# Equim-chan/Mortal

Hardware: AMD Instinct MI355X
Metric: env steps/sec (65536 parallel tables per GPU) (higher is better)
Workload: dtype u8/i32 state, f32 obs

## Files before the change

include/mortal_amd.h:

```cpp
#ifndef MORTAL_AMD_H
#define MORTAL_AMD_H

#include <stddef.h>
#include <stdint.h>

#ifdef __cplusplus
extern "C" {
#endif

typedef struct MjPool MjPool;

enum { MJ_DEAL_RAND08 = 0, MJ_DEAL_RAND09 = 1 };

const char* mj_last_error(void);
int mj_abi_version(void);

int mj_tables_upload(const void* payload, size_t size);

MjPool* mj_pool_create(int n_tables, int version, int deal_algo, int max_rows);
void mj_pool_destroy(MjPool* pool);

int mj_pool_reset(MjPool* pool, const uint64_t* nonces, const uint64_t* keys, const uint32_t* game_ids,
                  const uint8_t* agent_of_seat, int n_games_total);

// ... 15 lines not shown

int mj_replay_load(MjPool* pool, const uint64_t* script_host, const uint32_t* off_host, const uint8_t* tracked_host,
                   int n_logs, int always_include_kan_select, const uint64_t* nonces_host ,
                   const uint64_t* keys_host );
#define MJ_LOAD_DEAL_FROM_SEED 1
#define MJ_LOAD_AUGMENT 2
int mj_replay_load_pool(MjPool* dst, MjPool* src, int table0, const uint8_t* tracked_host ,
                        int always_include_kan_select, int flags , int64_t counts_out[3], void* stream);
int mj_replay_step(MjPool* pool, void* stream);
int mj_replay_meta(MjPool* pool, int32_t* meta_dev, void* stream);

int mj_table_apply_event(MjPool* pool, int table, const uint64_t* words_host, int n_words, void* stream);
int mj_table_mark_row(MjPool* pool, int table, int seat, int at_kan_select, void* stream);
int mj_table_query(MjPool* pool, int table, int seat, int what, const int32_t* args8_host, int32_t* out8_host, void* stream);

int mj_rows_count(MjPool* pool, int32_t n_rows_out[2], void* stream);
const uint32_t* mj_rows_dev(MjPool* pool, int agent);

int mj_encode(MjPool* pool, int agent, float* obs_dev, uint8_t* masks_dev, void* stream);
int mj_encode_oracle(MjPool* pool, int agent, float* out_dev, void* stream);
int mj_oracle_obs_rows(int version);
int mj_encode_timing(MjPool* pool, int enable, double* total_ms_out, int64_t* launches_out);
int mj_sp_timing(MjPool* pool, double* total_ms_out, int64_t* launches_out);
int mj_sp_phase_ticks(MjPool* pool, uint64_t* out8, void* stream);
int mj_pool_set_sp_schedule(MjPool* pool, int mode, int max_rows, int wide_grid, int min_level1, int min_level2);
int mj_sp_schedule_stats(MjPool* pool, uint64_t* out4, void* stream);

int mj_random_policy(MjPool* pool, int agent, const uint8_t* masks_dev, uint64_t seed, uint64_t cycle,
                     int32_t* actions_dev, void* stream);

int mj_greedy_policy(MjPool* pool, int agent, const uint8_t* masks_dev, const float* obs_dev, uint64_t seed, uint64_t cycle,
                     int32_t* actions_dev, void* stream);

int mj_counters(MjPool* pool, uint64_t out[8], void* stream);
int mj_results(MjPool* pool, int32_t* scores_out, uint8_t* done_out, void* stream);
#define MJ_STAT_FIELDS 44
enum MjStatField {
    MJ_ST_GAME = 0, MJ_ST_ROUND, MJ_ST_OYA, MJ_ST_POINT, MJ_ST_RANK_1, MJ_ST_RANK_2, MJ_ST_RANK_3, MJ_ST_RANK_4, MJ_ST_TOBI,
    MJ_ST_FUURO, MJ_ST_FUURO_NUM, MJ_ST_FUURO_POINT, MJ_ST_FUURO_AGARI, MJ_ST_FUURO_AGARI_JUN, MJ_ST_FUURO_AGARI_POINT,
    MJ_ST_FUURO_HOUJUU, MJ_ST_AGARI, MJ_ST_AGARI_AS_OYA, MJ_ST_AGARI_JUN, MJ_ST_AGARI_POINT_OYA, MJ_ST_AGARI_POINT_KO,
    MJ_ST_HOUJUU, MJ_ST_HOUJUU_JUN, MJ_ST_HOUJUU_TO_OYA, MJ_ST_HOUJUU_POINT_TO_OYA, MJ_ST_HOUJUU_POINT_TO_KO,
    MJ_ST_RIICHI, MJ_ST_RIICHI_AS_OYA, MJ_ST_RIICHI_JUN, MJ_ST_RIICHI_AGARI, MJ_ST_RIICHI_AGARI_POINT, MJ_ST_RIICHI_AGARI_JUN,
    MJ_ST_RIICHI_HOUJUU, MJ_ST_RIICHI_RYUKYOKU, MJ_ST_RIICHI_POINT, MJ_ST_CHASING_RIICHI, MJ_ST_RIICHI_GOT_CHASED,
    MJ_ST_DAMA_AGARI, MJ_ST_DAMA_AGARI_JUN, MJ_ST_DAMA_AGARI_POINT, MJ_ST_RYUKYOKU, MJ_ST_RYUKYOKU_POINT, MJ_ST_YAKUMAN,
    MJ_ST_NAGASHI_MANGAN
};
int mj_stat_logs(const uint64_t* words_host, const uint32_t* off_host , int n_logs,
// ... 66 lines not shown
```

mortal_amd/csrc/mj_capi.hip:

```cpp
#include <hip/hip_runtime.h>

#include <algorithm>
#include <cmath>
#include <cstdio>
#include <cstring>
#include <functional>
#include <memory>
#include <optional>
#include <string>
#include <vector>

#include "../../include/mortal_amd.h"
#include "mj_host.h"
#include "mj_step.hip"
#include "mj_replay.hip"
#include "mj_encode.hip"
#include "mj_sp.hip"
#include "mj_stat.hip"
#include "mj_gameplay.hip"
#include "mj_harvest.hip"

static_assert(sizeof(MjAlgoQuery) == 72, "MjAlgoQuery layout");
__global__ __launch_bounds__(64) void mj_k_algo_query(const MjAlgoQuery* q, int n, MjAlgoResult* out) {
    const int i = blockIdx.x * 64 + threadIdx.x;
// ... 692 lines not shown
    return kp;
}

static int sp_setup(MjPool* P, int agent, float* obs, hipStream_t s) {
    SpResources R;
    const PoolKnobs& K = P->knobs;
    if (R.err.alloc(SP_ERR_WORDS)) return -1;
    HIP_OK(hipMemset(R.err.get(), 0, SP_ERR_WORDS * sizeof(unsigned long long)));
    if (R.order.alloc(P->max_rows) || R.cls.alloc(P->max_rows)) return -1;
    R.grid = std::min(256 * SP_WGS, P->max_rows);
    if (K.sp_grid) R.grid = std::max(1, std::min(R.grid, *K.sp_grid));
    const bool env = !P->sp_sched_set;
    const int wide_mode = env && K.sp_wide ? *K.sp_wide : P->sp_wide_mode;
    const int wide_max_rows = env && K.sp_wide_max_rows ? *K.sp_wide_max_rows : P->sp_wide_max_rows;
    R.spare = wide_mode == 0 ? 0 : std::min(SP_PROMO_CAP, std::max(8, P->n_tables / 4) & ~1);
    if (wide_mode < 0 && P->n_tables > wide_max_rows) R.spare = 0;
    R.wide_areas = R.spare ? std::min(256, std::max(2, P->n_tables / 16)) : 0;
    const int areas = R.grid + R.spare + R.wide_areas;
    if (R.work.alloc(areas)) return -1;
    for (int g = 0; g < areas; g++) {
        SpWork& W = R.work.get()[g];
        HIP_OK(hipMemsetAsync(W.tag, 0, sizeof(W.tag), s));
        HIP_OK(hipMemsetAsync(&W.epoch, 0, sizeof(W.epoch) + sizeof(W.pad_), s));
    }
    if (R.queue.alloc(SP_Q_WORDS)) return -1;
    if (R.spare) {
        if (R.stream2.create_non_blocking() || R.ev_fork.create_no_timing() || R.ev_join.create_no_timing() || R.gaveup_host.alloc(1)) return -1;
        *R.gaveup_host.get() = 0ull;
        HIP_OK(hipMemsetAsync(R.queue.get(), 0, SP_Q_WORDS * sizeof(int), s));
        HIP_OK(hipStreamSynchronize(s));
        SpParams w = sp_params(P, R, agent, obs, 0);
        w.sweep = 1;
        hipLaunchKernelGGL(mj_k_sp_wide, dim3(1), dim3(SP_WIDE_THREADS), 0, s, w);
        hipLaunchKernelGGL(mj_k_sp_promo, dim3(1), dim3(SP_THREADS), 0, R.stream2.get(), w);
        HIP_OK(hipStreamSynchronize(R.stream2.get()));
        HIP_OK(hipStreamSynchronize(s));
        HIP_OK(hipGetLastError());
    }
    P->sp = std::move(R);
    P->sp_wide_mode = wide_mode;
    P->sp_wide_max_rows = wide_max_rows;
    if (env && K.sp_wide_grid) P->sp_wide_grid = std::max(1, *K.sp_wide_grid);
    if (env && K.sp_promo_min1) P->sp_promo_min[1] = std::max(1, *K.sp_promo_min1);
    if (env && K.sp_promo_min2) P->sp_promo_min[2] = std::max(1, *K.sp_promo_min2);
    return 0;
}
// ... 209 lines not shown
                    sp_[8], sp_[0], sp_[1], sp_[2], sp_[3], sp_[4], sp_[9], sp_[5], sp_[10], sp_[7]);
            for (int k = 11; k < 32; k++) fprintf(stderr, " %llu", sp_[k]);
            fprintf(stderr, "\n");
        }
    }
#endif
    if (!P) return fail("null pool");
    HIP_OK(hipStreamSynchronize((hipStream_t)stream));
    unsigned long long tmp[8];
    HIP_OK(hipMemcpy(tmp, P->counters.get(), sizeof tmp, hipMemcpyDeviceToHost));
    for (int i = 0; i < 8; i++) out[i] = tmp[i];
    out[5] = P->cycles;
    int f = 0;
    HIP_OK(hipMemcpy(&f, P->enc_flag.get(), sizeof f, hipMemcpyDeviceToHost));
    out[6] = (unsigned long long)f;
    if (P->sp.err) {
        unsigned long long e2[SP_ERR_WORDS];
        HIP_OK(hipMemcpy(e2, P->sp.err.get(), sizeof e2, hipMemcpyDeviceToHost));
        out[6] += e2[SP_ERR_OVERFLOW];
        out[7] = e2[SP_ERR_ROWS];
        const unsigned long long* pass = e2 + SP_ERR_PASS;
        if (P->knobs.sp_prof)
            fprintf(stderr, "[sp prof] rows %llu setup %llu expand %llu evalL0 %llu evalL>0 %llu encode %llu states %llu (wall_clock64 ticks, 100 MHz) | "
                    "expand passes: probes %llu lists+V %llu td-probes %llu layout %llu inserts %llu; items %llu expanded %llu edges %llu l0-entries %llu; level-0 probe %llu scoring %llu; workgroup lifetimes: sum %llu max %llu queue pops %llu hash resets %llu; eval wavefront time %llu; shader clock %.0f MHz (s_memtime cycles %llu over the lifetimes)\n",
                    e2[SP_ERR_ROWS], e2[SP_ERR_T_SETUP], e2[SP_ERR_T_EXPAND], e2[SP_ERR_T_EVAL0], e2[SP_ERR_T_EVAL], e2[SP_ERR_T_WRITE], e2[SP_ERR_STATES],
                    pass[0], pass[1], pass[2], pass[3], pass[4], pass[5], pass[6], e2[SP_ERR_EDGES], e2[SP_ERR_L0_ITEMS],
                    e2[SP_ERR_T_L0_PROBE], e2[SP_ERR_T_L0_SCORE], e2[SP_ERR_WG_LIFE], e2[SP_ERR_WG_LIFE_MAX], e2[SP_ERR_T_POP], e2[SP_ERR_T_RESET],
                    e2[SP_ERR_T_EVAL_WAVE], e2[SP_ERR_WG_LIFE] ? 100.0 * (double)e2[SP_ERR_WG_CLOCK] / (double)e2[SP_ERR_WG_LIFE] : 0.0,
                    e2[SP_ERR_WG_CLOCK]);
    }
    return 0;
}

#ifdef MJ_EMU
void mj_emu_sp_placed(uint64_t out[2]) { out[0] = g_sp_emu_placed[0]; out[1] = g_sp_emu_placed[1]; }
void mj_emu_sp_lost_claims(uint64_t out[4]) {
    for (int k = 0; k < 2; k++) out[k] = g_sp_emu_lost[2 + k], out[2 + k] = g_sp_emu_lost[k] - g_sp_emu_lost[2 + k];
}
#ifdef MJ_EMU_REGISTRY
void mj_emu_alloc_stats(uint64_t out[6]) {
    const emu::Registry& r = emu::R();
    out[0] = r.buffers.size(), out[1] = r.events.size(), out[2] = r.streams.size(), out[3] = r.bad_frees, out[4] = r.allocs, out[5] = r.syncs;
}
void mj_emu_fail_nth(int alloc, int sync) { emu::R().fail_alloc_in = alloc, emu::R().fail_sync_in = sync; }
#endif
#endif

int mj_sp_phase_ticks(MjPool* P, uint64_t out[8], void* stream) {
    if (!P) return fail("null pool");
    for (int i = 0; i < 8; i++) out[i] = 0;
    if (!P->sp.err) return 0;
    HIP_OK(hipStreamSynchronize((hipStream_t)stream));
    unsigned long long e2[8];
    HIP_OK(hipMemcpy(e2, P->sp.err.get(), sizeof e2, hipMemcpyDeviceToHost));
    for (int i = 0; i < 8; i++) out[i] = e2[i];
    return 0;
}

int mj_pool_set_sp_schedule(MjPool* P, int mode, int max_rows, int wide_grid, int min_level1, int min_level2) {
    if (!P) return fail("null pool");
    if (P->sp.work && mode != 0 && mode >= -1 && P->sp.spare == 0) return fail("mj_pool_set_sp_schedule: the work areas are allocated (call it before the first obs-v4 mj_encode)");
    if (mode >= -1) P->sp_wide_mode = mode > 0 ? 1 : mode;
    if (max_rows > 0) P->sp_wide_max_rows = max_rows;
    if (wide_grid > 0) P->sp_wide_grid = std::min(wide_grid, 256);
    if (min_level1 > 0) P->sp_promo_min[1] = min_level1;
    if (min_level2 > 0) P->sp_promo_min[2] = min_level2;
    P->sp_sched_set = true;
    return 0;
}

int mj_sp_schedule_stats(MjPool* P, uint64_t out[4], void* stream) {
    if (!P) return fail("null pool");
    for (int i = 0; i < 4; i++) out[i] = 0;
    if (!P->sp.err) return 0;
    HIP_OK(hipStreamSynchronize((hipStream_t)stream));
    unsigned long long e2[SP_ERR_WORDS];
    HIP_OK(hipMemcpy(e2, P->sp.err.get(), sizeof e2, hipMemcpyDeviceToHost));
    out[0] = P->sp_hybrid_launches;
// ... 462 lines not shown
```

mortal_amd/csrc/mj_sp.hip:

```cpp
#include <hip/hip_runtime.h>

#include <type_traits>
#ifdef MJ_EMU
#include <algorithm>
#endif

#include "mj_rules.h"
#include "mj_sptab.h"


#ifndef SP_THREADS
#define SP_THREADS 256
#endif
#define SP_CAP 16384
#define SP_T 17
#define SP_MAX_CAND 14
#ifndef SP_NS
#define SP_NS 16
#endif
#ifndef SP_SORT_MIN
#define SP_SORT_MIN 8
#endif
#ifndef SP_ITEM_CAP
#define SP_ITEM_CAP 64
#endif
#ifndef SP_WPS
#define SP_WPS 4
#endif
#define SP_WGS (4 * SP_WPS * 64 / SP_THREADS)

#ifndef SP_SET_BUCKETS
#define SP_SET_BUCKETS 1024
#endif
#define SP_SET_SLOTS (2 * SP_SET_BUCKETS)
#define SP_NODES (SP_CAP + SP_SET_SLOTS)
static_assert((SP_SET_BUCKETS & (SP_SET_BUCKETS - 1)) == 0 && SP_SET_BUCKETS >= 1 && SP_NODES <= (1 << 15), "slots are 15-bit fields");
#ifndef SP_TAIL_BATCH
#define SP_TAIL_BATCH 4
#endif
#define SP_Q_TAIL 32
#define SP_Q_PROMO_DONE 96
#define SP_PROMO_LEVELS 2
#define SP_Q_PROMO_ALLOC(p) (128 + 64 * (p))
#define SP_Q_PROMO_HEAD(p) (160 + 64 * (p))
#define SP_Q_PROMO_ENT 256
#ifndef SP_PROMO_CAP
#define SP_PROMO_CAP 512
#endif
#define SP_Q_WORDS (SP_Q_PROMO_ENT + SP_PROMO_CAP)
#ifndef SP_WIDE_THREADS
#define SP_WIDE_THREADS 1024
#endif
#define SP_POOL (SP_CAP * 32)
#define SP_ITEMS (SP_CAP * 4)
#define SP_L0_MAX 17
#define SP_EL_SLOT(v) ((v) & 0x7FFFu)
#define SP_EL_IDX(v) ((v) >> 15)
struct alignas(128) SpNode {
    float val[SP_T][3];
// ... 1 lines not shown
};
static_assert(sizeof(SpNode) == 256 && offsetof(SpNode, val) == 0, "SpNode layout");
struct alignas(16) SpHdr {
    u32 child_off;
    unsigned short n_ch;
    u8 sumreq, n_ent;
    u64 l0cnt2;
};
static_assert(sizeof(SpHdr) == 16 && offsetof(SpHdr, n_ch) == 4 && offsetof(SpHdr, sumreq) == 6 && offsetof(SpHdr, l0cnt2) == 8,
              "the evaluation reads the header as one or two u64");
struct SpKeys {
    u64 k0, k1, k2, k3;
    u64 dk;
};
#define SP_ENT_SLOT(e) ((e) & 0x7FFFu)
#define SP_ENT_KEY(e) (((e) >> 15) & 511u)
#define SP_ENT_LAST (1u << 24)
#define SP_ENT_COUNT(e) (((e) >> 25) & 7u)
#define SP_ENT_INVALID (1u << 28)
struct alignas(16) SpF4 { float x, y, z, w; };
#define SP_HANDOFF_WORDS 1024
struct alignas(128) SpWork {
    u64 tag[SP_CAP];
    SpNode node[SP_NODES];
    SpKeys keys[SP_CAP];
    SpHdr hdr[SP_CAP];
    u32 list[SP_CAP];
    u32 elist[SP_CAP];
    u32 pool[SP_POOL];
    u32 items[SP_ITEMS];
    SpF4 l0sc[SP_ITEMS];
    u32 epoch;
    u32 pad_[31];
    alignas(16) u32 handoff[SP_HANDOFF_WORDS];
#ifdef MJ_EMU
    u32 idx_of[SP_NODES];
#endif
};
static_assert(offsetof(SpWork, node) % 128 == 0 && sizeof(SpWork) % 128 == 0, "nodes on line boundaries");

#define SP_NT_ROWS 124
#define SP_NT_STRIDE (SP_T + 3)
__constant__ const float* c_sp_nt;
static inline void sp_not_tsumo_build(float* out ) {
    for (int n_left = 0; n_left < SP_NT_ROWS; n_left++)
        for (int q = 0; q < SP_NT_ROWS; q++) {
            float* r = out + ((size_t)n_left * SP_NT_ROWS + q) * SP_NT_STRIDE;
// ... 35 lines not shown
    SP_ERR_T_EVAL0 = 4,
    SP_ERR_T_EVAL = 5,
    SP_ERR_T_WRITE = 6,
    SP_ERR_STATES = 7,
    SP_ERR_PASS = 8,
    SP_ERR_EDGES = 15,
    SP_ERR_L0_ITEMS = 16,
    SP_ERR_T_L0_PROBE = 17,
    SP_ERR_T_L0_SCORE = 18,
    SP_ERR_WG_LIFE = 19,
    SP_ERR_WG_LIFE_MAX = 20,
    SP_ERR_T_POP = 21,
    SP_ERR_T_RESET = 22,
    SP_ERR_T_EVAL_WAVE = 23,
    SP_ERR_WG_CLOCK = 24,
    SP_ERR_STATS = 25,
    SP_ERR_WIDE_GAVEUP = 25,
    SP_ERR_PROMOTED = 26,
    SP_ERR_SWEPT = 27,
    SP_ERR_DUMP_T0 = 28,
    SP_ERR_DUMP_NARROW = 29,
    SP_ERR_DUMP_WIDE = 30,
    SP_ERR_DUMP_TAIL = 31,
    SP_ERR_WORDS = 32
};

__device__ static const float SP_URADORA[5][13] = {
    {0.639485f, 0.327801f, 0.0327134f, 0.f, 0.f, 0.f, 0.f, 0.f, 0.f, 0.f, 0.f, 0.f, 0.f},
    {0.406736f, 0.42281f, 0.147966f, 0.021674f, 0.0008142f, 0.f, 0.f, 0.f, 0.f, 0.f, 0.f, 0.f, 0.f},
    {0.257516f, 0.406819f, 0.246851f, 0.0757724f, 0.0122266f, 0.0008004f, 1.43e-5f, 0.f, 0.f, 0.f, 0.f, 0.f, 0.f},
    {0.162199f, 0.346513f, 0.301539f, 0.142396f, 0.0401276f, 0.0066491f, 0.0005575f, 1.85e-5f, 0.f, 0.f, 0.f, 0.f, 0.f},
    {0.101768f, 0.275319f, 0.313742f, 0.20189f, 0.081774f, 0.0215394f, 0.0035918f, 0.0003607f, 1.52e-5f, 3e-7f, 0.f, 0.f, 0.f}};
__device__ static const u8 SP_DISCARD_PRIO[38] = {
    6, 5, 4, 3, 2, 3, 4, 5, 6, 6, 5, 4, 3, 2, 3, 4, 5, 6, 6, 5, 4, 3, 2, 3, 4, 5, 6, 7, 7, 7, 7, 7, 7, 7, 1, 1, 1, 0};
constexpr __host__ __device__ int sp_discard_prio(int t) {
    return t < 27 ? 2 + (t % 9 > 4 ? t % 9 - 4 : 4 - t % 9) : t < 34 ? 7 : t < 37 ? 1 : 0;
}
constexpr bool sp_discard_prio_matches_table() {
    constexpr int tab[38] = {6, 5, 4, 3, 2, 3, 4, 5, 6, 6, 5, 4, 3, 2, 3, 4, 5, 6, 6, 5, 4, 3, 2, 3, 4, 5, 6, 7, 7, 7, 7, 7, 7, 7, 1, 1, 1, 0};
    for (int t = 0; t < 38; t++)
        if (sp_discard_prio(t) != tab[t]) return false;
    return true;
}
static_assert(sp_discard_prio_matches_table(), "sp_discard_prio != SP_DISCARD_PRIO");
MJD int sp_discard_key(int t) { return sp_discard_prio(t) * 64 + (63 - t); }
MJD int cmp_discard_priority(int l, int r) {
    int pl = SP_DISCARD_PRIO[l], pr = SP_DISCARD_PRIO[r];
// ... 76 lines not shown
    return *reinterpret_cast<const Tv*>(reinterpret_cast<const char*>(base) + byte_off);
#else
    return *reinterpret_cast<const SP_HBM Tv*>(reinterpret_cast<const SP_HBM char*>(base) + (unsigned long long)byte_off);
#endif
}
template <class Bp> __device__ __forceinline__ SpF4 sp_ld4(Bp base, u32 byte_off) {
#ifdef MJ_EMU
    return *reinterpret_cast<const SpF4*>(reinterpret_cast<const char*>(base) + byte_off);
#else
    const SP_HBM SpF4* p = reinterpret_cast<const SP_HBM SpF4*>(reinterpret_cast<const SP_HBM char*>(base) + (unsigned long long)byte_off);
    SpF4 r;
    r.x = p->x; r.y = p->y; r.z = p->z; r.w = p->w;
    return r;
#endif
}
struct SpF3 { float x, y, z; };
template <class Bp> __device__ __forceinline__ SpF3 sp_ld3(Bp base, u32 byte_off) {
#ifdef MJ_EMU
    return *reinterpret_cast<const SpF3*>(reinterpret_cast<const char*>(base) + byte_off);
#else
    const SP_HBM SpF3* p = reinterpret_cast<const SP_HBM SpF3*>(reinterpret_cast<const SP_HBM char*>(base) + (unsigned long long)byte_off);
    SpF3 r;
    r.x = p->x; r.y = p->y; r.z = p->z;
    return r;
#endif
}
template <class Bp> __device__ __forceinline__ void sp_st3(Bp base, u32 byte_off, float x, float y, float z) {
#ifdef MJ_EMU
    *reinterpret_cast<SpF3*>(reinterpret_cast<char*>(base) + byte_off) = SpF3{x, y, z};
#else
    SP_HBM SpF3* p = reinterpret_cast<SP_HBM SpF3*>(reinterpret_cast<SP_HBM char*>(base) + (unsigned long long)byte_off);
    p->x = x; p->y = y; p->z = z;
#endif
}
MJD int sp_f2i(float v) {
#if defined(MJ_EMU)
    return v != v ? 0 : v >= 2147483648.f ? 2147483647 : v <= -2147483648.f ? (-2147483647 - 1) : (int)v;
#else
    return (int)v;
#endif
}

MJD u64 sp_dk_add(u64 dk, int draw_tile, int discard_tile) {
    u32 d0 = (u32)dk & 63, d1 = (u32)(dk >> 6) & 63, d2 = (u32)(dk >> 12) & 63;
    u32 x0 = (u32)(dk >> 18) & 63, x1 = (u32)(dk >> 24) & 63, x2 = (u32)(dk >> 30) & 63, x3 = (u32)(dk >> 36) & 63;
    if (draw_tile >= 0) {
// ... 570 lines not shown
                Hand g = S.h;
                g.inc(t);
                kept = sp_keep_brute_dev(g, ld3, L - 1);
            } else {
                const u32 id1 = spt_id(TG, st, key1);
                const SpRec o1 = spt_opt(TG, ld3, (u32)C->r3[s][st], id1);
                u64 keepN = (u64)spt_keep_tiles(spt_rec(TG, st, key1, 1), o1) << (9 * st);
#pragma unroll
                for (int q = 0; q < 3; q++) {
                    const int u = q + (q >= st);
                    const u32 others = spt_merge(TG, (u32)C->r2[s][5 - sh_pair_idx(st, u)], id1);
                    const SpRec o = spt_opt(TG, ld3, others, (u32)C->id[s][u]);
                    keepN |= (u64)spt_keep_tiles(C->keep[s][u], o) << (9 * u);
                }
                const int yao = (int)((YAOKYUU_MASK >> t) & 1);
                SpCountSets cs;
                cs.c1 = C->cs[s][0];
                cs.c2 = C->cs[s][1];
                cs.nz = C->cs[s][2];
                kept = sp_keep_set(ld3, L - 1, spt_fin(o1), keepN, (int)C->cnt[s][0] + (hc == 1), (int)C->cnt[s][1] + (hc == 0),
                                   (int)C->cnt[s][2] + (yao && hc == 1), (int)C->cnt[s][3] + (yao && hc == 0), sp_count_sets_add(cs, t, hc));
            }
            kept &= ~(1ull << t);
            C->kept[tid] = kept;
        }
        if (prof) tp2 = wall_clock64();
        int n_entries;
        {
            const int wc = has_item ? S.w.get(my_t) : 0;
            const int nvar = has_item && sp_aka_in_wall(S, my_t) ? (wc >= 2 ? 2 : 1) : 1;
            const int nkeep = __popcll(kept), my_ent = nvar * nkeep;
            const u32 pv = sp_wave_scan_incl(has_item ? ((u32)my_ent | ((u32)wc << 16) | ((u32)(nkeep ? nvar : 0) << 24)) : 0u);
            const int sfn = __shfl((pre_ex - base) | (nt_lane << 16), has_item ? my_s : sb);
            const int s_first = sfn & 0xFFFF, s_n = sfn >> 16;
            const int s_last = s_first + s_n - 1;
            const u32 before = __shfl(pv, max(s_first - 1, 0)), upto = __shfl(pv, max(s_last, 0)), all = __shfl(pv, SP_NT - 1);
            const u32 base = s_first > 0 ? before : 0u;
            n_entries = (int)(all & 0xFFFFu);
            if (has_item) {
                C->coff[tid] = (unsigned short)(((pv - base) & 0xFFFFu) - (u32)my_ent);
                const int e_first = (int)((pv & 0xFFFFu) - (u32)my_ent);
                C->eoff[tid] = (unsigned short)e_first;
                {
                    int r = 0;
                    for (u64 rest = kept; rest; rest &= rest - 1, r++) {
                        const u32 d = (u32)(__ffsll((long long)rest) - 1);
// ... 156 lines not shown
        mj_team_sync<SP_NT>();
        if (prof) {
            tp4 = wall_clock64();
            acc_list += tp1 - tp0;
            acc_keep += tp2 - tp1;
            acc_layout += tp3 - tp2;
            acc_ins += tp4 - tp3;
            n_items_total += n_items;
            n_edges_total += n_entries;
        }
        sb = se;
    }
    if (prof && tid == 0) {
        atomicAdd(&X->pt[0], (unsigned long long)t_probe);
        atomicAdd(&X->pt[1], (unsigned long long)acc_list);
        atomicAdd(&X->pt[2], (unsigned long long)acc_keep);
        atomicAdd(&X->pt[3], (unsigned long long)acc_layout);
        atomicAdd(&X->pt[4], (unsigned long long)acc_ins);
        atomicAdd(&X->pt[5], (unsigned long long)n_items_total);
        atomicAdd(&X->pt[6], (unsigned long long)n);
    }
}

#define SP_EVAL_LDS_FLOATS(NT) (((NT) / 64) * 1408)

#define SP_EV_ENT 4
#define SP_EVW_WAVE_FLOATS 1408
MJD int sp_evw_team_floats(int T) { return SP_EV_ENT * (T + 4) * 4; }
__device__ static const u8 SP_EVW_STRIDE[SP_T + 1][4] = {
    {16, 16, 16, 16}, {20, 20, 20, 20}, {25, 25, 24, 24}, {29, 28, 29, 28}, {32, 32, 32, 32}, {37, 36, 38, 38}, {42, 41, 44, 41}, {44, 44, 44, 44},
    {48, 50, 50, 50}, {57, 56, 55, 54}, {58, 57, 56, 56}, {67, 66, 69, 60}, {68, 67, 66, 69}, {77, 68, 69, 70}, {78, 77, 76, 75}, {79, 78, 77, 76},
    {80, 86, 86, 85}, {97, 84, 86, 86}};
#define SP_EV0_STRIDE 28
#define SP_EV0_SC 20
#define SP_EV0_LAST 24

template <int TN>
__device__ SP_ATTR_EVAL0 void sp_eval_wave0(SpWork* W, SpCtx* X, float* WL, int first, int end, int stride, int lane_in_team, int off_,
                                           int team_in_wave, bool team_on) {
    SP_ASSUME_LDS(X);
    SP_ASSUME_LDS(WL);
    SP_HBM SpWork* const Wg = (SP_HBM SpWork*)sp_uniform(W);
    SP_HBM SpNode* const nodeB = sp_uniform(&Wg->node[0]);
    SP_HBM u32* const elistB = sp_uniform(&Wg->elist[0]);
    const int T = __builtin_amdgcn_readfirstlane(X->T), off = __builtin_amdgcn_readfirstlane(off_);
    const int ln = min(lane_in_team + off, SP_T - 1);
// ... 127 lines not shown
    static_assert(LK >= 1, "level 0 has no children: sp_eval_wave0");
    SP_ASSUME_LDS(X);
    SP_ASSUME_LDS(WL);
    SP_HBM SpWork* const Wg = (SP_HBM SpWork*)sp_uniform(W);
    const int T = __builtin_amdgcn_readfirstlane(X->T), off = __builtin_amdgcn_readfirstlane(off_);
    const int ln = min(lane_in_team + off, SP_T - 1);
    const int rows = T + 4;
    const int team_rows = __builtin_amdgcn_readfirstlane((int)SP_EVW_STRIDE[min(max(T, 0), SP_T)][min(max(off, 0), 3)]);
    float* const eb = WL + (team_on ? team_in_wave : 0) * (team_rows * 4);
    if (team_on)
        for (int r = lane_in_team; r < SP_EV_ENT * rows; r += T - off) *reinterpret_cast<SpF4*>(eb + 4 * r) = SpF4{0.f, 0.f, 0.f, 0.f};
    const float tp0 = X->tsumo_prob[0][ln], tp1 = X->tsumo_prob[1][ln], tp2 = X->tsumo_prob[2][ln], tp3 = X->tsumo_prob[3][ln];
    const SP_HBM float* const nt_rows = (const SP_HBM float*)c_sp_nt + (size_t)__builtin_amdgcn_readfirstlane(min(X->n_left, SP_NT_ROWS - 1)) * (SP_NT_ROWS * SP_NT_STRIDE);
    const int last = max(end - 1, 0);
    const u32 val_ln = (u32)offsetof(SpNode, val) + (u32)ln * 12u;
    SP_HBM SpNode* const nodeB = sp_uniform(&Wg->node[0]);
    SP_HBM u32* const elistB = sp_uniform(&Wg->elist[0]);
    SP_HBM u32* const poolB = sp_uniform(&Wg->pool[0]);
    SP_HBM SpHdr* const hdrB = sp_uniform(&Wg->hdr[0]);
    auto ld_slot = [&](int i) -> u32 { return sp_ld<u32>(elistB, 4u * (u32)min(i, last)); };
    auto ld_hdr = [&](u32 el) -> u64 { return sp_ld<unsigned long long>(hdrB, 16u * SP_EL_IDX(el)); };
    auto ld_m = [&](u64 hdr) -> float { return sp_ld<float>(nt_rows, 4u * ((u32)min((int)((hdr >> 48) & 0xFF), SP_NT_ROWS - 1) * SP_NT_STRIDE + (u32)ln)); };
    auto ld_ent = [&](u32 at) -> u32 { return sp_ld<u32>(poolB, 4u * min(at, (u32)(SP_POOL - 1))); };
    auto ld_val = [&](u32 ent) -> SpF3 { return sp_ld3(nodeB, SP_ENT_SLOT(ent) * (u32)sizeof(SpNode) + val_ln); };
    mj_team_sync<64>();

    int i = first;
    bool has = team_on && i < end;
    u32 s0 = ld_slot(i), s1 = ld_slot(i + stride), s2 = ld_slot(i + 2 * stride), s3 = ld_slot(i + 3 * stride);
    u64 h0 = ld_hdr(s0), h1 = ld_hdr(s1), h2 = ld_hdr(s2);
    float m_raw = ld_m(h0), m_nxt = ld_m(h1);
    u32 ent[SP_EV_ENT], entn[SP_EV_ENT], nent[SP_EV_ENT];
#pragma unroll
    for (int q = 0; q < SP_EV_ENT; q++) {
        ent[q] = ld_ent((u32)h0 + q);
        entn[q] = ld_ent((u32)h0 + SP_EV_ENT + q);
        nent[q] = ld_ent((u32)h1 + q);
    }
    SpF3 v[SP_EV_ENT];
#pragma unroll
    for (int q = 0; q < SP_EV_ENT; q++) v[q] = ld_val(ent[q]);

    int c0 = 0;
    float my_m = m_raw != 0.f ? m_raw : 1.f, my_r = sp_rcp_refined(my_m);
    float acc_t = 0.f, acc_w = 0.f, acc_e = 0.f;
    float nx_t = -3.40282347e+38f, nx_w = -3.40282347e+38f, nx_e = -3.40282347e+38f;
    int max_pack = -1;
    float* const row0 = eb + ln * 4;
    const int nl = T - ln;

    while (__ballot(has) != 0ull) {
        const int n_ch = (int)((h0 >> 32) & 0xFFFF);
        int k = 0, koff = 0;
#pragma unroll
        for (int q = 0; q < SP_EV_ENT; q++) {
            const u32 e = ent[q];
            const bool valid = has && c0 + q < n_ch;
            const bool bad = (e & SP_ENT_INVALID) != 0;
            if (valid && bad) X->overflow = 1;
            const int pack = (sp_f2i(v[q].z) << 9) | (int)SP_ENT_KEY(e);
#ifdef MJ_EMU
            if (valid && !bad && lane_in_team > 0 && ((unsigned)sp_f2i(v[q].z) >> 22)) X->overflow = 1;
#endif
            const bool better = valid && !bad && pack > max_pack;
            nx_t = better ? v[q].x : nx_t;
            nx_w = better ? v[q].y : nx_w;
            nx_e = better ? v[q].z : nx_e;
            max_pack = better ? pack : max_pack;
            if (valid && (e & SP_ENT_LAST)) {
                const u32 cnt = SP_ENT_COUNT(e);
                const float tpc = cnt <= 1 ? tp0 : cnt == 2 ? tp1 : cnt == 3 ? tp2 : tp3;
                float* row = row0 + koff;
                row[0] = nx_t;
                row[1] = nx_w;
                row[2] = nx_e;
                row[7] = tpc * m_raw;
                k++;
                koff += rows * 4;
                nx_t = nx_w = nx_e = -3.40282347e+38f;
                max_pack = -1;
            }
        }
        c0 += SP_EV_ENT;
        const bool done = has && c0 >= n_ch;
        u32 up[SP_EV_ENT], upn[SP_EV_ENT], nent2[SP_EV_ENT];
        SpF3 vn[SP_EV_ENT];
        const u32 up_off = done ? (u32)h1 + SP_EV_ENT : (u32)h0 + (u32)c0 + SP_EV_ENT;
#pragma unroll
        for (int q = 0; q < SP_EV_ENT; q++) up[q] = done ? nent[q] : entn[q];
#pragma unroll
        for (int q = 0; q < SP_EV_ENT; q++) vn[q] = ld_val(up[q]);
#pragma unroll
        for (int q = 0; q < SP_EV_ENT; q++) upn[q] = ld_ent(up_off + q);
        float m_n2 = 0.f;
        u64 h3 = 0ull;
        u32 s4 = 0u;
// ... 319 lines not shown
            for (int i = 0; i < 5; i++) X.dora_ind[i] = i < X.n_dora ? F1(dora_ind, i) : T_UNK;
            int nf = 0;
            if (!(X.is_menzen && F1(ankan_n, p) == 0)) {
                int fn = F1(fuuro_n, p);
                for (int k = 0; k < fn; k++)
                    for (int j = 0; j < 4; j++) {
                        int t = F3(fuuro, p, k, j);
                        if (t != MJ_NONE) nf += dora_factor(L, deaka(t)) + (is_aka(t) ? 1 : 0);
                    }
                int na = F1(ankan_n, p);
                for (int k = 0; k < na; k++) {
                    int t = F2(ankan, p, k);
                    nf += 4 * dora_factor(L, t) + ((t == T_5M || t == T_5P || t == T_5S) ? 1 : 0);
                }
            }
            X.num_doras_in_fuuro = nf & 0xFF;
            X.prefer_riichi = F1(scores, p) >= 1000;
            X.calc_double_riichi = can_discard0 && (F1(pflags, p) & PF_CAN_W_RIICHI) != 0;
            X.calc_haitei = calc_haitei;
            X.T = T;
            X.n_left = n_left;
            X.n_list = 0;
            X.n_pool = 0;
            X.overflow = 0;
            X.prof = prof;
            for (int k = 0; k < 8; k++) X.pt[k] = 0;
            for (int l = 0; l < 5; l++) X.lvl_begin[l] = X.lvl_end[l] = 0;
        }
        if (with_probs) {
            for (int q = tid; q < 4 * SP_T; q += NT) {
                int i = q / SP_T, j = q % SP_T;
                X.tsumo_prob[i][j] = j < T ? (float)(i + 1) / (float)(n_left - j) : 0.f;
            }
        }

        const SpTabG TG = sp_tab_g(c_sp_tab);
        if (tid >= SPEC && tid < SPEC + 34) {
            const int d = tid - SPEC;
            if (can_discard) {
                if (root.h.get(d)) {
                    Hand hc = root.h;
                    hc.dec(d);
                    X.spec_req[0][d] = sp_req_of_hand(TG, c_mj_tables, hc, ld3, cur_shanten);
                    if (cur_shanten > 3) X.spec_req[1][d] = sp_req_of_hand(TG, c_mj_tables, hc, ld3, cur_shanten + 1);
                }
            } else if (d == 0) {
// ... 196 lines not shown
#define SP_ACQUIRE_AGENT() ((void)0)
#define SP_SPIN_PAUSE() ((void)0)
#endif

#ifdef SP_ROWDUMP
#define SP_DUMP(P) ((P).rowdump != nullptr)
#else
#define SP_DUMP(P) false
#endif
template <int NT>
struct SpLds {
    union Teams {
        TableOne st;
        SpChunk wchunk[NT / SP_NT];
        float ev[SP_EVAL_LDS_FLOATS(NT)];
        SpWaveArea wave[NT / 64];
    };
};

template <int NT, bool WIDE, bool PROMO>
__device__ __forceinline__ void sp_kernel_body(SpParams P) {
    __shared__ SpCtx X;
    __shared__ int s_row, s_k;
    __shared__ unsigned long long s_stat[SP_ERR_STATS];
    if (threadIdx.x < SP_ERR_STATS) s_stat[threadIdx.x] = 0ull;
    __shared__ typename SpLds<NT>::Teams s_tm;
    constexpr bool LDS_SET = !WIDE && !PROMO;
    __shared__ __attribute__((aligned(16))) u64 s_set[SP_SET_SLOTS];
    for (int i = threadIdx.x; i < SP_SET_SLOTS; i += NT) s_set[i] = 0ull;
    unsigned n_graph_rows = 0;
    SpWork* W = WIDE ? P.work + P.n_narrow + P.promo_cap + blockIdx.x : P.work + blockIdx.x;
    SpWork* const W_own = W;
    const int tid_wg = threadIdx.x, tid = tid_wg;

    unsigned tag_epoch = W->epoch;
    unsigned own_epoch = tag_epoch;
    bool main_done = false, drained = false;

    const long long t_wg_in = SP_DUMP(P) ? wall_clock64() : 0;
    const long long t_wg0 = P.prof ? wall_clock64() : 0;
#ifndef MJ_EMU
    const long long c_wg0 = P.prof ? clock64() : 0;
#endif
    long long t_pop = 0, t_reset = 0;
    const int n_heavy = P.n_rows - P.queue[1 + 7];
    bool wave_mode = false;
    for (;;) {
        const int tid = SP_OPQ(2, tid_wg);
// ... 157 lines not shown
                                    SpHandoff* H = reinterpret_cast<SpHandoff*>(W->handoff);
                                    H->R = R;
                                    H->row = row;
                                    H->next_lv = lv;
                                    W->epoch = tag_epoch;
                                    if (SP_DUMP(P)) P.rowdump[(size_t)row * 12 + 8] = (uint32_t)t_0, P.rowdump[(size_t)row * 12 + 9] = (uint32_t)wall_clock64();
                                }
                            }
                            SP_DRAIN_STORES();
                            __syncthreads();
                            if (tid == 0) {
                                SP_RELEASE_AGENT();
                                __hip_atomic_store(P.queue + SP_Q_PROMO_ENT + pq * (SP_PROMO_CAP / SP_PROMO_LEVELS) + k, (int)(W - P.work) + 1, __ATOMIC_RELAXED,
                                                   __HIP_MEMORY_SCOPE_AGENT);
                            }
                            W = P.work + gridDim.x + pq * (P.promo_cap / SP_PROMO_LEVELS) + k;
                            tag_epoch = W->epoch;
                            parked = true;
                            break;
                        }
                    }
                }
                const int ns = min(SP_NS, max(1, (e - b + NT / SP_NT - 1) / (NT / SP_NT)));
                for (int c0 = b + ns * (tid / SP_NT); c0 < e; c0 += ns * (NT / SP_NT))
                    sp_expand_chunk<LDS_SET>(W, &X, &s_tm.wchunk[tid / SP_NT], c0, min(ns, e - c0), lv);
                __syncthreads();
                if (tid == 0) {
                    X.lvl_begin[lv - 1] = e;
                    X.lvl_end[lv - 1] = min(X.n_list, SP_CAP);
                }
                __syncthreads();
            }
            t_2 = wall_clock64();
#ifdef MJ_EMU
            if (tid == 0 && !parked) sp_emu_check_unique(W, &X);
#endif
            if (!parked)
            for (int lv = 0; lv <= cur_shanten; lv++) {
                const int b = X.lvl_begin[lv], e = X.lvl_end[lv];
                if (lv == 0) {
                    if (tid == 0) X.n_items = 0;
                    __syncthreads();
                    const int ns = min(SP_NS, max(1, (e - b + NT / SP_NT - 1) / (NT / SP_NT)));
                    for (int c0 = b + ns * (tid / SP_NT); c0 < e; c0 += ns * (NT / SP_NT))
                        sp_l0_probe_chunk(W, &X, &s_tm.wchunk[tid / SP_NT], c0, min(ns, e - c0));
                    __syncthreads();
                    const long long t_2a = wall_clock64();
                    const int n_items = min(X.n_items, SP_ITEMS);
                    if ((tid & ~63) < n_items) sp_l0_score_all(W, &X, n_items, tid, NT);
                    __syncthreads();
                    if (P.prof && tid == 0) {
                        X.pt[7] += (unsigned long long)(t_2a - t_2);
                        s_stat[SP_ERR_T_L0_SCORE] += (unsigned long long)(wall_clock64() - t_2a);
                    }
                }
                sp_sort_level<NT>(W, reinterpret_cast<int*>(s_tm.ev), b, e);
                {
                    const int off = min(cur_shanten - lv, T - 1), TW = T - off;
                    const int wl = tid & 63, tw = wl / TW, ln = wl - tw * TW;
                    float* wl_lds = s_tm.ev + (tid >> 6) * SP_EVW_WAVE_FLOATS;
                    const long long t_ev0 = P.prof ? wall_clock64() : 0;
// ... 14 lines not shown
                            if (lv == 1) sp_eval_wave<8, 1>(W, &X, wl_lds, b + team2, e, n_teams2, ln, off, tw, on);
                            else sp_eval_wave<8, 2>(W, &X, wl_lds, b + team2, e, n_teams2, ln, off, tw, on);
                        } else if (T <= 16) {
                            if (lv == 1) sp_eval_wave<16, 1>(W, &X, wl_lds, b + team2, e, n_teams2, ln, off, tw, on);
                            else sp_eval_wave<16, 2>(W, &X, wl_lds, b + team2, e, n_teams2, ln, off, tw, on);
                        } else {
                            if (lv == 1) sp_eval_wave<17, 1>(W, &X, wl_lds, b + team2, e, n_teams2, ln, off, tw, on);
                            else sp_eval_wave<17, 2>(W, &X, wl_lds, b + team2, e, n_teams2, ln, off, tw, on);
                        }
                    }
                    if (P.prof && (tid & 63) == 0) atomicAdd(&s_stat[SP_ERR_T_EVAL_WAVE], (unsigned long long)(wall_clock64() - t_ev0));
                }
                __syncthreads();
                if (lv == 0) t_3 = wall_clock64();
            }
            t_4 = wall_clock64();
        }

        if (!parked) sp_row_write<false, NT>(W->node, X, R, tid, out, s_tm.ev);
        __syncthreads();
        if (tid == 0) {
            long long t_5 = wall_clock64();
            if (!parked) s_stat[SP_ERR_ROWS] += 1ull;
            s_stat[SP_ERR_T_SETUP] += (unsigned long long)(t_1 - t_0);
            if (with_probs) {
                s_stat[SP_ERR_T_EXPAND] += (unsigned long long)(t_2 - t_1);
                if (!parked) {
                    s_stat[SP_ERR_T_EVAL0] += (unsigned long long)(t_3 - t_2);
                    s_stat[SP_ERR_T_EVAL] += (unsigned long long)(t_4 - t_3);
                    s_stat[SP_ERR_T_WRITE] += (unsigned long long)(t_5 - t_4);
                    s_stat[SP_ERR_STATES] += (unsigned long long)X.n_list;
                    s_stat[SP_ERR_EDGES] += (unsigned long long)X.n_pool;
                    s_stat[SP_ERR_L0_ITEMS] += (unsigned long long)X.n_items;
                }
                if (P.prof)
                    for (int k = 0; k < 7; k++) s_stat[SP_ERR_PASS + k] += X.pt[k];
                if (P.prof) s_stat[SP_ERR_T_L0_PROBE] += X.pt[7];
            }
            if (SP_DUMP(P) && !parked) {
                uint32_t* d = P.rowdump + (size_t)row * 12;
                int nreq = 0;
                for (int c = 0; c < n_cand; c++) nreq += X.cand_nreq[c];
                d[0] = (uint32_t)(WIDE ? 0x40000000 | (promoted ? 0x20000000 : 0) : s_row); d[1] = (uint32_t)(cur_shanten | T << 8 | n_cand << 16 | (int)can_discard << 24); d[2] = (uint32_t)nreq;
                d[3] = with_probs ? (uint32_t)X.n_list : 0u; d[4] = with_probs ? (uint32_t)X.n_pool : 0u; d[5] = with_probs ? (uint32_t)X.n_items : 0u;
                d[6] = (uint32_t)(t_5 - t_0);
                if (!promoted) d[8] = (uint32_t)t_0, d[9] = 0u;
// ... 16 lines not shown
            W->epoch = tag_epoch;
            if (PROMO && P.promo_cap > 0) {
                SP_DRAIN_STORES();
                __hip_atomic_fetch_add(P.queue + SP_Q_PROMO_DONE, 1, __ATOMIC_RELAXED, __HIP_MEMORY_SCOPE_AGENT);
            }
        }
    }
    if (P.prof && tid == 0) {
        const unsigned long long life = (unsigned long long)(wall_clock64() - t_wg0);
        s_stat[SP_ERR_WG_LIFE] += life;
#ifndef MJ_EMU
        s_stat[SP_ERR_WG_CLOCK] += (unsigned long long)(clock64() - c_wg0);
#endif
        atomicMax(&P.err[SP_ERR_WG_LIFE_MAX], life);
        s_stat[SP_ERR_T_POP] += (unsigned long long)t_pop;
        s_stat[SP_ERR_T_RESET] += (unsigned long long)t_reset;
    }
    __syncthreads();
    if (SP_DUMP(P) && tid == 0) {
        atomicMin(&P.err[SP_ERR_DUMP_T0], (unsigned long long)t_wg_in);
        atomicMax(&P.err[WIDE ? SP_ERR_DUMP_WIDE : SP_ERR_DUMP_NARROW], (unsigned long long)wall_clock64());
    }
    if (tid < SP_ERR_STATS && tid != SP_ERR_WG_LIFE_MAX && s_stat[tid]) atomicAdd(&P.err[tid], s_stat[tid]);
    if constexpr (!WIDE) {
    if (wave_mode) {
        const int wv = tid >> 6, lane = tid & 63;
        unsigned long long w_rows = 0, w_ticks = 0, w_over = 0;
        for (;;) {
            int q = 0;
            if (lane == 0) q = n_heavy + atomicAdd(P.queue + SP_Q_TAIL, SP_TAIL_BATCH);
            q = __shfl(q, 0);
            if (q >= P.n_rows) break;
            const int qe = min(q + SP_TAIL_BATCH, P.n_rows);
            for (; q < qe; q++) {
                const unsigned long long r = sp_light_row(P.rows, P.snap, P.obs, W, &s_tm.wave[wv], (int)P.order[q]);
                w_rows++;
                w_ticks += r & 0x7FFFFFFFFFFFFFFFull;
                w_over += r >> 63;
            }
        }
        if (lane == 0 && w_rows) {
            atomicAdd(&P.err[SP_ERR_ROWS], w_rows);
            atomicAdd(&P.err[SP_ERR_T_SETUP], w_ticks);
            if (w_over) atomicAdd(&P.err[SP_ERR_OVERFLOW], w_over);
        }
        if (SP_DUMP(P) && lane == 0) atomicMax(&P.err[SP_ERR_DUMP_TAIL], (unsigned long long)wall_clock64());
// ... 8 lines not shown
```

mortal_amd/pool.py:

```python
import ctypes as C

import numpy as np
import torch

from . import tables
from ._lib import MortalAmdError, check, lib

OBS_ROWS = {1: 938, 2: 942, 3: 934, 4: 1012}
ACTION_SPACE = 46
DEAL_RAND08, DEAL_RAND09 = 0, 1


def default_deal_algo():
    import os

    v = os.environ.get("MORTAL_AMD_DEAL_ALGO", "rand09").strip().lower()
    if v in ("0", "rand08", "rand0.8", "0.8"):
        return DEAL_RAND08
    if v in ("1", "rand09", "rand0.9", "0.9", "0.9.1"):
        return DEAL_RAND09
    raise ValueError(f"MORTAL_AMD_DEAL_ALGO={v!r}: expected rand08 or rand09")

_tables_ready = False

# ... 360 lines not shown
        scores = np.zeros((self.n_games_total, 4), dtype=np.int32)
        done = np.zeros(self.n_games_total, dtype=np.uint8)
        check(self._L.mj_results(self.h, scores.ctypes.data, done.ctypes.data, self._stream()))
        return scores, done

    def first_error(self):
        t = C.c_int(-1)
        code = check(self._L.mj_pool_first_error(self.h, C.byref(t), self._stream()))
        return code, t.value

    def encode_timing(self, enable=True):
        ms = C.c_double(0)
        n = C.c_int64(0)
        check(self._L.mj_encode_timing(self.h, int(enable), C.byref(ms), C.byref(n)))
        return ms.value, n.value

    def sp_timing(self):
        ms = C.c_double(0)
        n = C.c_int64(0)
        check(self._L.mj_sp_timing(self.h, C.byref(ms), C.byref(n)))
        return ms.value, n.value

    def sp_phase_ticks(self):
        out = (C.c_uint64 * 8)()
        check(self._L.mj_sp_phase_ticks(self.h, out, self._stream()))
        return dict(zip(("overflow", "rows", "setup", "expand", "level0", "eval", "write", "states"), (int(x) for x in out)))

    def set_sp_schedule(self, mode=-2, max_rows=0, wide_grid=0, min_level1=0, min_level2=0):
        check(self._L.mj_pool_set_sp_schedule(self.h, mode, max_rows, wide_grid, min_level1, min_level2))

    def sp_schedule_stats(self):
        out = (C.c_uint64 * 4)()
        check(self._L.mj_sp_schedule_stats(self.h, out, self._stream()))
        return dict(zip(("hybrid_launches", "rows_promoted", "rows_swept", "wide_gave_up"), (int(x) for x in out)))

    def debug_table(self, table):
        size = self._L.mj_debug_table_size()
        buf = (C.c_uint8 * size)()
        check(self._L.mj_debug_table(self.h, table, buf, size, self._stream()))
        raw = bytes(buf)
        out = {}
        for ent in self._L.mj_debug_layout().decode().strip(";").split(";"):
            name, size, count, off = ent.split(":")
            size, count, off = int(size), int(count), int(off)
            dt = {1: np.uint8, 2: np.uint16, 4: np.int32, 8: np.uint64}[size]
            out[name] = np.frombuffer(raw, dtype=dt, count=count, offset=off).copy()
        return out


# ... 7 lines not shown
```

Measured before the change: 4.449 million.

## Short-circuit dead leaf expansion at max tsumo depth via shared zero node

When level 1 is the last tsumo level (T equals current shanten), children can never reach a win. Instead of the full sp_expand_chunk, a lightweight dead-chunk expander points every child entry at a shared zero-initialised node slot, and level-0 evaluation is skipped for such rows. For LK==1 the eval also loads two floats instead of three and skips writing the unused first field. The change adds a counter for these rows and a ninth profiling output, and depends on the zero slot staying zero and on the claim that those leaves contribute nothing.

```diff
diff --git a/include/mortal_amd.h b/include/mortal_amd.h
--- a/include/mortal_amd.h
+++ b/include/mortal_amd.h
@@ -61,7 +61,7 @@
 int mj_oracle_obs_rows(int version);
 int mj_encode_timing(MjPool* pool, int enable, double* total_ms_out, int64_t* launches_out);
 int mj_sp_timing(MjPool* pool, double* total_ms_out, int64_t* launches_out);
-int mj_sp_phase_ticks(MjPool* pool, uint64_t* out8, void* stream);
+int mj_sp_phase_ticks(MjPool* pool, uint64_t* out9, void* stream);
 int mj_pool_set_sp_schedule(MjPool* pool, int mode, int max_rows, int wide_grid, int min_level1, int min_level2);
 int mj_sp_schedule_stats(MjPool* pool, uint64_t* out4, void* stream);
 
diff --git a/mortal_amd/csrc/mj_capi.hip b/mortal_amd/csrc/mj_capi.hip
--- a/mortal_amd/csrc/mj_capi.hip
+++ b/mortal_amd/csrc/mj_capi.hip
@@ -738,6 +738,7 @@
         SpWork& W = R.work.get()[g];
         HIP_OK(hipMemsetAsync(W.tag, 0, sizeof(W.tag), s));
         HIP_OK(hipMemsetAsync(&W.epoch, 0, sizeof(W.epoch) + sizeof(W.pad_), s));
+        HIP_OK(hipMemsetAsync(&W.node[SP_ZERO_SLOT], 0, sizeof(SpNode), s));
     }
     if (R.queue.alloc(SP_Q_WORDS)) return -1;
     if (R.spare) {
@@ -993,12 +994,12 @@
         const unsigned long long* pass = e2 + SP_ERR_PASS;
         if (P->knobs.sp_prof)
             fprintf(stderr, "[sp prof] rows %llu setup %llu expand %llu evalL0 %llu evalL>0 %llu encode %llu states %llu (wall_clock64 ticks, 100 MHz) | "
-                    "expand passes: probes %llu lists+V %llu td-probes %llu layout %llu inserts %llu; items %llu expanded %llu edges %llu l0-entries %llu; level-0 probe %llu scoring %llu; workgroup lifetimes: sum %llu max %llu queue pops %llu hash resets %llu; eval wavefront time %llu; shader clock %.0f MHz (s_memtime cycles %llu over the lifetimes)\n",
+                    "expand passes: probes %llu lists+V %llu td-probes %llu layout %llu inserts %llu; items %llu expanded %llu edges %llu l0-entries %llu; level-0 probe %llu scoring %llu; workgroup lifetimes: sum %llu max %llu queue pops %llu hash resets %llu; eval wavefront time %llu; shader clock %.0f MHz (s_memtime cycles %llu over the lifetimes); dead-leaf rows %llu\n",
                     e2[SP_ERR_ROWS], e2[SP_ERR_T_SETUP], e2[SP_ERR_T_EXPAND], e2[SP_ERR_T_EVAL0], e2[SP_ERR_T_EVAL], e2[SP_ERR_T_WRITE], e2[SP_ERR_STATES],
                     pass[0], pass[1], pass[2], pass[3], pass[4], pass[5], pass[6], e2[SP_ERR_EDGES], e2[SP_ERR_L0_ITEMS],
                     e2[SP_ERR_T_L0_PROBE], e2[SP_ERR_T_L0_SCORE], e2[SP_ERR_WG_LIFE], e2[SP_ERR_WG_LIFE_MAX], e2[SP_ERR_T_POP], e2[SP_ERR_T_RESET],
                     e2[SP_ERR_T_EVAL_WAVE], e2[SP_ERR_WG_LIFE] ? 100.0 * (double)e2[SP_ERR_WG_CLOCK] / (double)e2[SP_ERR_WG_LIFE] : 0.0,
-                    e2[SP_ERR_WG_CLOCK]);
+                    e2[SP_ERR_WG_CLOCK], e2[SP_ERR_DEAD_LEAF]);
     }
     return 0;
 }
@@ -1017,14 +1018,15 @@
 #endif
 #endif
 
-int mj_sp_phase_ticks(MjPool* P, uint64_t out[8], void* stream) {
-    if (!P) return fail("null pool");
-    for (int i = 0; i < 8; i++) out[i] = 0;
+int mj_sp_phase_ticks(MjPool* P, uint64_t out[9], void* stream) {
+    if (!P) return fail("null pool");
+    for (int i = 0; i < 9; i++) out[i] = 0;
     if (!P->sp.err) return 0;
     HIP_OK(hipStreamSynchronize((hipStream_t)stream));
-    unsigned long long e2[8];
+    unsigned long long e2[SP_ERR_WORDS];
     HIP_OK(hipMemcpy(e2, P->sp.err.get(), sizeof e2, hipMemcpyDeviceToHost));
     for (int i = 0; i < 8; i++) out[i] = e2[i];
+    out[8] = e2[SP_ERR_DEAD_LEAF];
     return 0;
 }
 
diff --git a/mortal_amd/csrc/mj_sp.hip b/mortal_amd/csrc/mj_sp.hip
--- a/mortal_amd/csrc/mj_sp.hip
+++ b/mortal_amd/csrc/mj_sp.hip
@@ -34,7 +34,8 @@
 #endif
 #define SP_SET_SLOTS (2 * SP_SET_BUCKETS)
 #define SP_NODES (SP_CAP + SP_SET_SLOTS)
-static_assert((SP_SET_BUCKETS & (SP_SET_BUCKETS - 1)) == 0 && SP_SET_BUCKETS >= 1 && SP_NODES <= (1 << 15), "slots are 15-bit fields");
+#define SP_ZERO_SLOT SP_NODES
+static_assert((SP_SET_BUCKETS & (SP_SET_BUCKETS - 1)) == 0 && SP_SET_BUCKETS >= 1 && SP_ZERO_SLOT < (1 << 15), "slots are 15-bit fields");
 #ifndef SP_TAIL_BATCH
 #define SP_TAIL_BATCH 4
 #endif
@@ -82,7 +83,7 @@
 #define SP_HANDOFF_WORDS 1024
 struct alignas(128) SpWork {
     u64 tag[SP_CAP];
-    SpNode node[SP_NODES];
+    SpNode node[SP_NODES + 1];
     SpKeys keys[SP_CAP];
     SpHdr hdr[SP_CAP];
     u32 list[SP_CAP];
@@ -164,7 +165,8 @@
     SP_ERR_DUMP_NARROW = 29,
     SP_ERR_DUMP_WIDE = 30,
     SP_ERR_DUMP_TAIL = 31,
-    SP_ERR_WORDS = 32
+    SP_ERR_DEAD_LEAF = 32,
+    SP_ERR_WORDS = 33
 };
 
 __device__ static const float SP_URADORA[5][13] = {
@@ -287,6 +289,17 @@
     const SP_HBM SpF3* p = reinterpret_cast<const SP_HBM SpF3*>(reinterpret_cast<const SP_HBM char*>(base) + (unsigned long long)byte_off);
     SpF3 r;
     r.x = p->x; r.y = p->y; r.z = p->z;
+    return r;
+#endif
+}
+struct SpF2 { float x, y; };
+template <class Bp> __device__ __forceinline__ SpF2 sp_ld2(Bp base, u32 byte_off) {
+#ifdef MJ_EMU
+    return *reinterpret_cast<const SpF2*>(reinterpret_cast<const char*>(base) + byte_off);
+#else
+    const SP_HBM SpF2* p = reinterpret_cast<const SP_HBM SpF2*>(reinterpret_cast<const SP_HBM char*>(base) + (unsigned long long)byte_off);
+    SpF2 r;
+    r.x = p->x; r.y = p->y;
     return r;
 #endif
 }
@@ -903,6 +916,9 @@
                                    (int)C->cnt[s][2] + (yao && hc == 1), (int)C->cnt[s][3] + (yao && hc == 0), sp_count_sets_add(cs, t, hc));
             }
             kept &= ~(1ull << t);
+#ifdef MJ_EMU
+            if (L == 1 && kept == 0ull) X->overflow = 1;
+#endif
             C->kept[tid] = kept;
         }
         if (prof) tp2 = wall_clock64();
@@ -1105,6 +1121,53 @@
     }
 }
 
+__device__ __noinline__ void sp_expand_dead_chunk(SpWork* W, SpCtx* X, SpChunk* C, int first, int n) {
+    SP_ASSUME_LDS(X);
+    SP_ASSUME_LDS(C);
+    SP_HBM SpWork* const Wg = (SP_HBM SpWork*)W;
+    const SpTabG TG = sp_tab_g(*SP_OPQ_PTR(1, &c_sp_tab));
+    const bool prof = X->prof != nullptr;
+    const long long tq0 = prof ? wall_clock64() : 0;
+    sp_chunk_probe(Wg, X, C, TG, first, n, 1);
+    const int s = threadIdx.x & (SP_NT - 1);
+    if (s < n) {
+        const SpState S = sp_chunk_state(C, s);
+        const u64 req = C->req[s];
+        int total = 0, sumreq = 0;
+        for (u64 rest = req; rest; rest &= rest - 1) {
+            const int t = __ffsll((long long)rest) - 1, wc = S.w.get(t);
+            total += sp_aka_in_wall(S, t) && wc >= 2 ? 2 : 1;
+            sumreq += wc;
+        }
+        int base = 0;
+        if (total) {
+            base = atomicAdd(&X->n_pool, total);
+            if (base + total > SP_POOL) { X->overflow = 1; base = SP_POOL; total = 0; }
+        }
+        int e = 0;
+        for (u64 rest = req; rest; rest &= rest - 1) {
+            const int t = __ffsll((long long)rest) - 1, wc = S.w.get(t);
+            const bool aka = sp_aka_in_wall(S, t);
+            for (int variant = 0; variant < 2; variant++) {
+                if (variant == 0 ? (aka && wc < 2) : !aka) continue;
+                const int count = !aka ? wc : variant == 0 ? wc - 1 : 1;
+                if (e < total && base + e < SP_POOL) Wg->pool[base + e] = (u32)SP_ZERO_SLOT | SP_ENT_LAST | ((u32)count << 25);
+                e++;
+            }
+        }
+        SP_HBM SpHdr& hd = Wg->hdr[first + s];
+        hd.child_off = total ? (u32)min(base, SP_POOL - 1) : 0u;
+        hd.n_ch = (unsigned short)total;
+        hd.sumreq = (u8)(sumreq & 0xFF);
+        hd.n_ent = (u8)min(total, 255);
+    }
+    mj_team_sync<SP_NT>();
+    if (prof && s == 0) {
+        atomicAdd(&X->pt[0], (unsigned long long)(wall_clock64() - tq0));
+        atomicAdd(&X->pt[6], (unsigned long long)n);
+    }
+}
+
 #define SP_EVAL_LDS_FLOATS(NT) (((NT) / 64) * 1408)
 
 #define SP_EV_ENT 4
@@ -1278,7 +1341,15 @@
     auto ld_hdr = [&](u32 el) -> u64 { return sp_ld<unsigned long long>(hdrB, 16u * SP_EL_IDX(el)); };
     auto ld_m = [&](u64 hdr) -> float { return sp_ld<float>(nt_rows, 4u * ((u32)min((int)((hdr >> 48) & 0xFF), SP_NT_ROWS - 1) * SP_NT_STRIDE + (u32)ln)); };
     auto ld_ent = [&](u32 at) -> u32 { return sp_ld<u32>(poolB, 4u * min(at, (u32)(SP_POOL - 1))); };
-    auto ld_val = [&](u32 ent) -> SpF3 { return sp_ld3(nodeB, SP_ENT_SLOT(ent) * (u32)sizeof(SpNode) + val_ln); };
+    auto ld_val = [&](u32 ent) -> SpF3 {
+        const u32 at = SP_ENT_SLOT(ent) * (u32)sizeof(SpNode) + val_ln;
+        if constexpr (LK == 1) {
+            const SpF2 p = sp_ld2(nodeB, at + 4u);
+            return SpF3{0.f, p.x, p.y};
+        } else {
+            return sp_ld3(nodeB, at);
+        }
+    };
     mj_team_sync<64>();
 
     int i = first;
@@ -1319,7 +1390,7 @@
             if (valid && !bad && lane_in_team > 0 && ((unsigned)sp_f2i(v[q].z) >> 22)) X->overflow = 1;
 #endif
             const bool better = valid && !bad && pack > max_pack;
-            nx_t = better ? v[q].x : nx_t;
+            if constexpr (LK != 1) nx_t = better ? v[q].x : nx_t;
             nx_w = better ? v[q].y : nx_w;
             nx_e = better ? v[q].z : nx_e;
             max_pack = better ? pack : max_pack;
@@ -1327,7 +1398,7 @@
                 const u32 cnt = SP_ENT_COUNT(e);
                 const float tpc = cnt <= 1 ? tp0 : cnt == 2 ? tp1 : cnt == 3 ? tp2 : tp3;
                 float* row = row0 + koff;
-                row[0] = nx_t;
+                if constexpr (LK != 1) row[0] = nx_t;
                 row[1] = nx_w;
                 row[2] = nx_e;
                 row[7] = tpc * m_raw;
@@ -1693,6 +1764,7 @@
             X.n_left = n_left;
             X.n_list = 0;
             X.n_pool = 0;
+            X.n_items = 0;
             X.overflow = 0;
             X.prof = prof;
             for (int k = 0; k < 8; k++) X.pt[k] = 0;
@@ -1935,8 +2007,8 @@
 __device__ __forceinline__ void sp_kernel_body(SpParams P) {
     __shared__ SpCtx X;
     __shared__ int s_row, s_k;
-    __shared__ unsigned long long s_stat[SP_ERR_STATS];
-    if (threadIdx.x < SP_ERR_STATS) s_stat[threadIdx.x] = 0ull;
+    __shared__ unsigned long long s_stat[SP_ERR_STATS + 1];
+    if (threadIdx.x <= SP_ERR_STATS) s_stat[threadIdx.x] = 0ull;
     __shared__ typename SpLds<NT>::Teams s_tm;
     constexpr bool LDS_SET = !WIDE && !PROMO;
     __shared__ __attribute__((aligned(16))) u64 s_set[SP_SET_SLOTS];
@@ -2140,8 +2212,13 @@
                     }
                 }
                 const int ns = min(SP_NS, max(1, (e - b + NT / SP_NT - 1) / (NT / SP_NT)));
-                for (int c0 = b + ns * (tid / SP_NT); c0 < e; c0 += ns * (NT / SP_NT))
-                    sp_expand_chunk<LDS_SET>(W, &X, &s_tm.wchunk[tid / SP_NT], c0, min(ns, e - c0), lv);
+                if (__builtin_expect(lv == 1 && T == cur_shanten, 0)) {
+                    for (int c0 = b + ns * (tid / SP_NT); c0 < e; c0 += ns * (NT / SP_NT))
+                        sp_expand_dead_chunk(W, &X, &s_tm.wchunk[tid / SP_NT], c0, min(ns, e - c0));
+                } else {
+                    for (int c0 = b + ns * (tid / SP_NT); c0 < e; c0 += ns * (NT / SP_NT))
+                        sp_expand_chunk<LDS_SET>(W, &X, &s_tm.wchunk[tid / SP_NT], c0, min(ns, e - c0), lv);
+                }
                 __syncthreads();
                 if (tid == 0) {
                     X.lvl_begin[lv - 1] = e;
@@ -2150,11 +2227,12 @@
                 __syncthreads();
             }
             t_2 = wall_clock64();
+            t_3 = t_2;
 #ifdef MJ_EMU
             if (tid == 0 && !parked) sp_emu_check_unique(W, &X);
 #endif
             if (!parked)
-            for (int lv = 0; lv <= cur_shanten; lv++) {
+            for (int lv = (cur_shanten >= 1 && T == cur_shanten) ? 1 : 0; lv <= cur_shanten; lv++) {
                 const int b = X.lvl_begin[lv], e = X.lvl_end[lv];
                 if (lv == 0) {
                     if (tid == 0) X.n_items = 0;
@@ -2215,6 +2293,7 @@
         if (tid == 0) {
             long long t_5 = wall_clock64();
             if (!parked) s_stat[SP_ERR_ROWS] += 1ull;
+            if (!parked && with_probs && cur_shanten >= 1 && T == cur_shanten) s_stat[SP_ERR_STATS] += 1ull;
             s_stat[SP_ERR_T_SETUP] += (unsigned long long)(t_1 - t_0);
             if (with_probs) {
                 s_stat[SP_ERR_T_EXPAND] += (unsigned long long)(t_2 - t_1);
@@ -2277,6 +2356,7 @@
         atomicMax(&P.err[WIDE ? SP_ERR_DUMP_WIDE : SP_ERR_DUMP_NARROW], (unsigned long long)wall_clock64());
     }
     if (tid < SP_ERR_STATS && tid != SP_ERR_WG_LIFE_MAX && s_stat[tid]) atomicAdd(&P.err[tid], s_stat[tid]);
+    if (tid == SP_ERR_STATS && s_stat[tid]) atomicAdd(&P.err[SP_ERR_DEAD_LEAF], s_stat[tid]);
     if constexpr (!WIDE) {
     if (wave_mode) {
         const int wv = tid >> 6, lane = tid & 63;
diff --git a/mortal_amd/pool.py b/mortal_amd/pool.py
--- a/mortal_amd/pool.py
+++ b/mortal_amd/pool.py
@@ -406,9 +406,9 @@
         return ms.value, n.value
 
     def sp_phase_ticks(self):
-        out = (C.c_uint64 * 8)()
+        out = (C.c_uint64 * 9)()
         check(self._L.mj_sp_phase_ticks(self.h, out, self._stream()))
-        return dict(zip(("overflow", "rows", "setup", "expand", "level0", "eval", "write", "states"), (int(x) for x in out)))
+        return dict(zip(("overflow", "rows", "setup", "expand", "level0", "eval", "write", "states", "dead_leaf_rows"), (int(x) for x in out)))
 
     def set_sp_schedule(self, mode=-2, max_rows=0, wide_grid=0, min_level1=0, min_level2=0):
         check(self._L.mj_pool_set_sp_schedule(self.h, mode, max_rows, wide_grid, min_level1, min_level2))
```

Result: faster. 4.500 million, median of 6 (+1.1%).
